# Lemnon95/multithreading_string_matching

Measured on AMD Instinct MI355X. Metric: payload GB/s scanned + matches/s, 1M x 1500B pkts, 1 pattern, higher is better.
Workload: dtype u8; 1 GPU; 1000000 synthetic 1500 B UDP payloads per GPU (a..z, NUL-free, seed 1234), one 16-byte pattern planted in ~10% of packets; BASELINE configs[1]; packets_per_gpu=1000000, payload_len=1500, patterns=1, pattern_len=16, parallelism=packets sharded over 1 GPU(s), all-reduce(SUM) of counts

## Files before the change

multithreading_string_matching_amd/csrc/kmp_dev_common.h:

```cpp
#ifndef KMP_DEV_COMMON_H
#define KMP_DEV_COMMON_H

#include <hip/hip_runtime.h>
#include <stdint.h>

#include "kmp_device.h"

namespace {

constexpr uint32_t ONES  = 0x01010101u;
constexpr uint32_t HIGHS = 0x80808080u;

__device__ __forceinline__ uint32_t zero_byte_mask(uint32_t x) { return (x - ONES) & ~x & HIGHS; }

__device__ __forceinline__ uint32_t wave_shl1(uint32_t v, uint32_t fill)
{
    return (uint32_t)__builtin_amdgcn_update_dpp((int)fill, (int)v, 0x130, 0xF, 0xF, false);
}

__device__ __forceinline__ uint32_t sgpr(uint32_t v) { return (uint32_t)__builtin_amdgcn_readfirstlane((int)v); }

template <bool MASKED>
__device__ __forceinline__ bool is_cand(uint32_t d, uint32_t first, uint32_t mask)
{
    return MASKED ? (((d ^ first) & mask) == 0u) : (d == first);
}
typedef uint32_t u32x4 __attribute__((ext_vector_type(4)));


template <int N>
__device__ __forceinline__ void ring_wait(u32x4 &a, u32x4 &b)
{
    asm volatile("s_waitcnt vmcnt(%2)" : "+v"(a), "+v"(b) : "i"(N) : "memory");
    __builtin_amdgcn_sched_barrier(0);
}

__device__ __forceinline__ void kmp_step(uint32_t ch, uint32_t &j, uint32_t m, const uint8_t *pat,
                                         const uint8_t *fail, uint32_t &cnt)
{
    while (j > 0u && pat[j] != ch) j = fail[j - 1u];
    if (pat[j] == ch) ++j;
    if (j == m) { ++cnt; j = fail[m - 1u]; }
}

__device__ __forceinline__ uint64_t ballot64(bool p) { return __builtin_amdgcn_ballot_w64(p); }

typedef int32_t i32x4 __attribute__((ext_vector_type(4)));

__device__ __forceinline__ i32x4 make_rsrc(const uint8_t *base, uint32_t bytes)
{
    const uint64_t p = reinterpret_cast<uint64_t>(base);
    i32x4 r;
    r.x = (int32_t)sgpr((uint32_t)p);
    r.y = (int32_t)sgpr((uint32_t)(p >> 32) & 0xFFFFu);
    r.z = (int32_t)sgpr(bytes);
    r.w = 0x00020000;
    return r;
}

template <bool NT, bool FRESH = false, bool SAME_REGS = false>
__device__ __forceinline__ void flat_issue(u32x4 &dst, i32x4 rsrc, uint32_t vo, uint32_t so)
{
    if (SAME_REGS) {
        if (NT) asm volatile("s_nop 4\n\tbuffer_load_dwordx4 %0, %1, %2, %3 offen nt" : "+v"(dst) : "v"(vo), "s"(rsrc), "s"(so) : "memory");
        else    asm volatile("s_nop 4\n\tbuffer_load_dwordx4 %0, %1, %2, %3 offen" : "+v"(dst) : "v"(vo), "s"(rsrc), "s"(so) : "memory");
    } else if (FRESH) {
        if (NT) asm volatile("s_nop 4\n\tbuffer_load_dwordx4 %0, %1, %2, %3 offen nt" : "=v"(dst) : "v"(vo), "s"(rsrc), "s"(so) : "memory");
        else    asm volatile("s_nop 4\n\tbuffer_load_dwordx4 %0, %1, %2, %3 offen" : "=v"(dst) : "v"(vo), "s"(rsrc), "s"(so) : "memory");
    } else {
        if (NT) asm volatile("buffer_load_dwordx4 %0, %1, %2, %3 offen nt" : "=v"(dst) : "v"(vo), "s"(rsrc), "s"(so) : "memory");
        else    asm volatile("buffer_load_dwordx4 %0, %1, %2, %3 offen" : "=v"(dst) : "v"(vo), "s"(rsrc), "s"(so) : "memory");
    }
}

struct PatConst {
    uint32_t m;
    uint32_t p[4];
};

__device__ __forceinline__ PatConst load_pat_const(const kmp_pattern_dev *gp)
{
    PatConst pc;
    pc.m = gp->m;
#pragma unroll
    for (int d = 0; d < 4; ++d) pc.p[d] = reinterpret_cast<const uint32_t *>(gp->pat)[d];
    asm volatile("" : "+s"(pc.m), "+s"(pc.p[0]), "+s"(pc.p[1]), "+s"(pc.p[2]), "+s"(pc.p[3]));
    return pc;
}

struct Emitter {
    uint4              *out;
    unsigned long long *counter;
    unsigned long long  cap;
    uint32_t            pattern;
    unsigned long long *marks;
    uint32_t            mark_stride;
    uint32_t            mark_rows;
    const uint2        *windows;
    uint32_t            win_first;
    uint32_t            win_last;
};
static_assert(sizeof(Emitter) % 16 == 0, "the kernel arguments behind the Emitter keep their alignment");

__device__ __forceinline__ void mark_match_as(bool ok, uint64_t pkt, uint32_t pattern, const Emitter &e)
{
    const uint32_t lane = threadIdx.x & 63u;
    uint64_t b = ballot64(ok);
    while (b != 0ull) {
        const uint32_t l = (uint32_t)__builtin_ctzll(b);
        const uint32_t pl = (uint32_t)__builtin_amdgcn_readlane((int)pattern, (int)l);
        const uint32_t klo = (uint32_t)__builtin_amdgcn_readlane((int)(uint32_t)pkt, (int)l);
        const uint32_t khi = (uint32_t)__builtin_amdgcn_readlane((int)(uint32_t)(pkt >> 32), (int)l);
        const uint64_t k = ((uint64_t)khi << 32) | klo;
        b &= ~ballot64(ok && pattern == pl && pkt == k);
        if (lane == l && pl < e.mark_rows && (k >> 6) < e.mark_stride)
            atomicOr(e.marks + (uint64_t)pl * e.mark_stride + (k >> 6), 1ull << (k & 63u));
    }
}

__device__ __forceinline__ void emit_filtered(bool ok, uint64_t pkt, uint32_t offset, uint32_t pattern, const Emitter &e)
{
    if (e.marks) { mark_match_as(ok, pkt, pattern, e); return; }
    const uint64_t b = ballot64(ok);
    if (b == 0ull) return;
    const uint32_t leader = (uint32_t)__builtin_ctzll(b);
    const uint32_t lane = threadIdx.x & 63u;
    unsigned long long base = 0ull;
    if (lane == leader) base = atomicAdd(e.counter, (unsigned long long)__builtin_popcountll(b));
    const uint32_t blo = (uint32_t)__builtin_amdgcn_readlane((int)(uint32_t)base, (int)leader);
    const uint32_t bhi = (uint32_t)__builtin_amdgcn_readlane((int)(uint32_t)(base >> 32), (int)leader);
    if (ok) {
        const uint32_t rank = __builtin_amdgcn_mbcnt_hi((uint32_t)(b >> 32), __builtin_amdgcn_mbcnt_lo((uint32_t)b, 0u));
        const unsigned long long slot = (((unsigned long long)bhi << 32) | blo) + rank;
        if (slot < e.cap) e.out[slot] = make_uint4((uint32_t)pkt, (uint32_t)(pkt >> 32), offset, pattern);
    }
}

template <bool EMIT>
__device__ __forceinline__ void emit_match_as(bool ok, uint64_t pkt, uint32_t offset, uint32_t pattern, const Emitter &e)
{
    if (!EMIT) return;
    if (e.windows) {
        uint2 win = make_uint2(0u, 0u);
        if (ok) win = e.windows[pattern];
        ok = ok && win.x <= offset && offset <= win.y;
    }
    emit_filtered(ok, pkt, offset, pattern, e);
}

template <bool EMIT>
__device__ __forceinline__ void emit_match(bool ok, uint64_t pkt, uint32_t offset, const Emitter &e)
{
    if (!EMIT) return;
    if (e.windows) ok = ok && e.win_first <= offset && offset <= e.win_last;
    emit_filtered(ok, pkt, offset, e.pattern, e);
}

__device__ __forceinline__ int32_t nul_limit(int32_t maxi, const uint32_t (&w)[5], uint64_t zl, uint64_t st, bool dead_in, uint32_t lane)
{
    const uint64_t below = (1ull << lane) - 1ull;
    const uint64_t st_le = st & (below | (1ull << lane));
    bool nul_before;
    if (st_le == 0ull) nul_before = dead_in || ((zl & below) != 0ull);
    else {
        const uint32_t sl = 63u - (uint32_t)__builtin_clzll(st_le);
        nul_before = (zl & below & ~((1ull << sl) - 1ull)) != 0ull;
    }
    const uint32_t m0 = zero_byte_mask(w[0]), m1 = zero_byte_mask(w[1]), m2 = zero_byte_mask(w[2]), m3 = zero_byte_mask(w[3]);
    uint32_t zi = 16u;
    if (m3) zi = 12u + ((uint32_t)__builtin_ctz(m3) >> 3);
    if (m2) zi = 8u + ((uint32_t)__builtin_ctz(m2) >> 3);
    if (m1) zi = 4u + ((uint32_t)__builtin_ctz(m1) >> 3);
    if (m0) zi = (uint32_t)__builtin_ctz(m0) >> 3;
    return nul_before ? -1 : min(maxi, (int32_t)zi - 1);
}

__device__ __forceinline__ uint32_t pk_min_u16(uint32_t a, uint32_t b)
{
    uint32_t r;
    asm("v_pk_min_u16 %0, %1, %2" : "=v"(r) : "v"(a), "v"(b));
    return r;
}
__device__ __forceinline__ uint32_t pk_max_u16(uint32_t a, uint32_t b)
{
    uint32_t r;
    asm("v_pk_max_u16 %0, %1, %2" : "=v"(r) : "v"(a), "v"(b));
    return r;
}
__device__ __forceinline__ uint32_t pk_add_u16(uint32_t a, uint32_t b)
{
    uint32_t r;
    asm("v_pk_add_u16 %0, %1, %2" : "=v"(r) : "v"(a), "v"(b));
    return r;
}
__device__ __forceinline__ uint32_t pk_rsub_sat_u16(uint32_t k, uint32_t b)
{
    uint32_t r;
    asm("v_pk_sub_u16 %0, %1, %2 clamp" : "=v"(r) : "s"(k), "v"(b));
    return r;
}
__device__ __forceinline__ uint32_t zero_half_mask(uint32_t x) { return (x - 0x00010001u) & ~x & 0x80008000u; }

__device__ __forceinline__ uint64_t mqsad(uint32_t lo, uint32_t hi, uint32_t ref, uint64_t acc)
{
    return __builtin_amdgcn_mqsad_pk_u16_u8(((uint64_t)hi << 32) | lo, ref, acc);
}

__device__ __forceinline__ uint32_t filter_sad(const uint32_t (&w)[5], uint32_t first, uint64_t (&S)[4], uint32_t (&t)[4])
{
#pragma unroll
    for (int q = 0; q < 4; ++q) {
        S[q] = mqsad(w[q], w[q + 1], first, 0ull);
        t[q] = pk_min_u16((uint32_t)S[q], (uint32_t)(S[q] >> 32));
    }
    return pk_min_u16(pk_min_u16(t[0], t[1]), pk_min_u16(t[2], t[3]));
}

__device__ __forceinline__ uint32_t halves_product(uint32_t x)
{
    uint32_t r;
    asm("v_mul_u32_u24_sdwa %0, %1, %1 dst_sel:DWORD dst_unused:UNUSED_PAD src0_sel:WORD_0 src1_sel:WORD_1" : "=v"(r) : "v"(x));
    return r;
}

template <bool EMIT>
__device__ __forceinline__ uint32_t tally_group(int q, uint64_t Sq, bool barred, uint32_t nv2, uint32_t found, uint32_t p0, uint32_t &cnt, uint64_t pkt,
                                                const Emitter &em)
{
    uint32_t lo = (uint32_t)Sq, hi = (uint32_t)(Sq >> 32);
    if (barred) {
        asm volatile("" ::: "memory");
        lo = pk_max_u16(lo, pk_rsub_sat_u16((uint32_t)(4 * q + 1) | ((uint32_t)(4 * q + 2) << 16), nv2));
        hi = pk_max_u16(hi, pk_rsub_sat_u16((uint32_t)(4 * q + 3) | ((uint32_t)(4 * q + 4) << 16), nv2));
    }
    if (!EMIT) return pk_add_u16(found, pk_add_u16(pk_rsub_sat_u16(0x00010001u, lo), pk_rsub_sat_u16(0x00010001u, hi)));
#pragma unroll
    for (int a = 0; a < 4; ++a) {
        const bool ok = (((a < 2 ? lo : hi) >> (16 * (a & 1))) & 0xFFFFu) == 0u;
        cnt += ok ? 1u : 0u;
        emit_match<EMIT>(ok, pkt, p0 + (uint32_t)(4 * q + a), em);
    }
    return found;
}

template <int ND, bool EMIT>
__device__ __forceinline__ void confirm_block0(uint64_t (&S)[4], const uint32_t (&t)[4], const uint32_t (&c)[8], bool barred, uint32_t nv2, uint32_t p0,
                                               const PatConst &pc, bool more, uint32_t &cnt, uint64_t pkt, const Emitter &em, bool (&on)[4])
{
    uint32_t found = 0u;
#pragma unroll
    for (int q = 0; q < 4; ++q) {
        on[q] = ballot64(halves_product(t[q]) == 0u) != 0ull;
        if (!on[q]) continue;
        asm volatile("" ::: "memory");
        if (ND > 1) {
            S[q] = mqsad(c[q + 1], c[q + 2], pc.p[1], S[q]);
            S[q] = mqsad(c[q + 2], c[q + 3], pc.p[2], S[q]);
            S[q] = mqsad(c[q + 3], c[q + 4], pc.p[3], S[q]);
        }
        if (more) continue;
        found = tally_group<EMIT>(q, S[q], barred, nv2, found, p0, cnt, pkt, em);
    }
    if (!EMIT) cnt += (found & 0xFFFFu) + (found >> 16);
}

template <bool EMIT>
__device__ __forceinline__ void confirm_sad(uint64_t (&S)[4], const uint32_t (&t)[4], const uint32_t (&w)[5], uint4 v, u32x4 bn, uint32_t fz, int32_t maxi,
                                            uint32_t p0, const PatConst &pc, const kmp_pattern_dev *gp, uint32_t &cnt, uint64_t pkt,
                                            const Emitter &em)
{
    const uint32_t m = pc.m;
    const bool barred = ballot64(maxi < 15 && fz != 0u) != 0ull;
    uint32_t nv2 = 0u;
    if (barred) {
        if (ballot64(maxi >= 0) == 0ull) return;
        const uint32_t nv = (uint32_t)min(max(maxi + 1, 0), 16);
        nv2 = nv | (nv << 16);
    }
    uint32_t c[8] = {w[0], w[1], w[2], w[3], w[4], 0u, 0u, 0u};
    bool on[4];
    if (m <= 4u) { confirm_block0<1, EMIT>(S, t, c, barred, nv2, p0, pc, false, cnt, pkt, em, on); return; }
    c[5] = wave_shl1(v.y, sgpr(bn.y)); c[6] = wave_shl1(v.z, sgpr(bn.z)); c[7] = wave_shl1(v.w, sgpr(bn.w));
    const bool more = m > 16u;
    confirm_block0<4, EMIT>(S, t, c, barred, nv2, p0, pc, more, cnt, pkt, em, on);
    if (!more) return;

    for (uint32_t k = 1u; 16u * k < m; ++k) {
        uint32_t mn = 0xFFFFFFFFu;
#pragma unroll
        for (int q = 0; q < 4; ++q)
            if (on[q]) mn = pk_min_u16(mn, pk_min_u16((uint32_t)S[q], (uint32_t)(S[q] >> 32)));
        if (ballot64(halves_product(mn) == 0u) == 0ull) return;
        const uint4 pk = reinterpret_cast<const uint4 *>(gp->pat)[k];
        const uint32_t left = m - 16u * k;
#pragma unroll
        for (int j = 0; j < 4; ++j) c[j] = c[j + 4];
        c[4] = wave_shl1(c[4], (uint32_t)__builtin_amdgcn_readlane((int)bn.x, (int)k));
        c[5] = wave_shl1(c[5], (uint32_t)__builtin_amdgcn_readlane((int)bn.y, (int)k));
        c[6] = wave_shl1(c[6], (uint32_t)__builtin_amdgcn_readlane((int)bn.z, (int)k));
        c[7] = wave_shl1(c[7], (uint32_t)__builtin_amdgcn_readlane((int)bn.w, (int)k));
#pragma unroll
        for (int q = 0; q < 4; ++q) {
            if (!on[q]) continue;
            asm volatile("" ::: "memory");
            S[q] = mqsad(c[q], c[q + 1], pk.x, S[q]);
            if (left > 4u)  { asm volatile("" ::: "memory"); S[q] = mqsad(c[q + 1], c[q + 2], pk.y, S[q]); }
            if (left > 8u)  { asm volatile("" ::: "memory"); S[q] = mqsad(c[q + 2], c[q + 3], pk.z, S[q]); }
            if (left > 12u) { asm volatile("" ::: "memory"); S[q] = mqsad(c[q + 3], c[q + 4], pk.w, S[q]); }
        }
    }
    uint32_t found = 0u;
#pragma unroll
    for (int q = 0; q < 4; ++q) {
        if (!on[q]) continue;
        asm volatile("" ::: "memory");
        found = tally_group<EMIT>(q, S[q], barred, nv2, found, p0, cnt, pkt, em);
    }
    if (!EMIT) cnt += (found & 0xFFFFu) + (found >> 16);
}


struct kmp_plan_entry { uint64_t k; uint64_t off; };

}

#endif
```

multithreading_string_matching_amd/csrc/kmp_scan_stream.hip:

```cpp
#include <hip/hip_runtime.h>
#include <stdint.h>

#include <algorithm>

#include "kmp_device.h"
#include "kmp_launch.h"
#include "kmp_dev_common.h"

namespace {


__global__ void __launch_bounds__(KMP_BLOCK_THREADS)
kmp_build_bitmap_kernel(const uint64_t *__restrict__ pkt_off, uint64_t n, unsigned long long *__restrict__ bitmap)
{
    for (uint64_t k = (uint64_t)blockIdx.x * blockDim.x + threadIdx.x; k < n; k += (uint64_t)gridDim.x * blockDim.x) {
        const uint64_t slot = pkt_off[k] >> 4;
        atomicOr(bitmap + (slot >> 6), 1ull << (slot & 63ull));
    }
}

__global__ void __launch_bounds__(KMP_BLOCK_THREADS)
kmp_plan_kernel(const uint64_t *__restrict__ pkt_off, const uint32_t *__restrict__ pkt_len, uint64_t n, uint64_t nwaves,
                kmp_plan_shape shape, kmp_plan_entry *__restrict__ plan)
{
    const uint64_t w = (uint64_t)blockIdx.x * blockDim.x + threadIdx.x;
    if (w > nwaves) return;
    const uint64_t l16 = ((uint64_t)pkt_len[n - 1] + 15ull) & ~15ull;
    const uint64_t end = pkt_off[n - 1] + (l16 < 16ull ? 16ull : l16);
    if (w == nwaves) { plan[w].k = n; plan[w].off = end; return; }
    uint64_t target = pkt_off[0];
    if (shape.units == 0u) target += w * shape.step;
    else {
        const uint64_t r = w / shape.units, u = w % shape.units;
        const uint64_t in = u <= shape.big_units ? u * shape.step : shape.big_units * shape.step + (u - shape.big_units) * shape.small;
        target += r * shape.region + (in < shape.region ? in : shape.region);
    }
    uint64_t lo = 0, hi = n;
    while (lo < hi) {
        const uint64_t mid = (lo + hi) >> 1;
        if (pkt_off[mid] < target) lo = mid + 1; else hi = mid;
    }
    if (lo > 0 && w > 0) {
        const uint64_t next = (lo < n) ? pkt_off[lo] : end;
        if (next >= target && target - pkt_off[lo - 1] < next - target) --lo;
    }
    plan[w].k = lo;
    plan[w].off = (lo < n) ? pkt_off[lo] : end;
}

#define KMP_WHOLE false
#define KMP_FLAT_KERNEL kmp_scan_flat_kernel
#define KMP_PACKED_KERNEL kmp_scan_packed_kernel
#include "kmp_scan_stream_kernels.inc"
#undef KMP_WHOLE
#undef KMP_FLAT_KERNEL
#undef KMP_PACKED_KERNEL
#define KMP_WHOLE true
#define KMP_FLAT_KERNEL kmp_scan_flat_whole_kernel
#define KMP_PACKED_KERNEL kmp_scan_packed_whole_kernel
#include "kmp_scan_stream_kernels.inc"
#undef KMP_WHOLE
#undef KMP_FLAT_KERNEL
#undef KMP_PACKED_KERNEL

}

namespace {
Emitter emitter_of(const kmp_scan_args &a)
{
    Emitter e{};
    e.out = reinterpret_cast<uint4 *>(a.emit_out);
    e.counter = a.emit_counter;
    e.cap = a.emit_cap;
    e.pattern = 0;
    e.marks = a.emit_marks;
    e.mark_stride = a.mark_stride;
    e.mark_rows = a.mark_rows;
    e.windows = reinterpret_cast<const uint2 *>(a.emit_windows);
    e.win_first = 0u;
    e.win_last = 0xFFFFFFFFu;
    return e;
}

template <int DEPTH>
hipError_t launch_flat_t(const kmp_scan_args &a, hipStream_t st)
{
    dim3 grid(a.blocks_x, a.n_ids), block(KMP_BLOCK_THREADS);
    const Emitter em = emitter_of(a);
#define KMP_FLAT_ARGS a.arena, a.n_pkts, a.uniform_stride, a.uniform_len, a.pkts_per_wave, a.patterns, a.pat_ids, a.partials, a.zero_counts, em
    if (a.whole) {
        if (kmp_emits(a))
            hipLaunchKernelGGL((kmp_scan_flat_whole_kernel<4, true, true>), grid, block, 0, st, KMP_FLAT_ARGS);
        else if (a.nontemporal)
            hipLaunchKernelGGL((kmp_scan_flat_whole_kernel<4, true>), grid, block, 0, st, KMP_FLAT_ARGS);
        else
            hipLaunchKernelGGL((kmp_scan_flat_whole_kernel<4, false>), grid, block, 0, st, KMP_FLAT_ARGS);
    } else if (kmp_emits(a))
        hipLaunchKernelGGL((kmp_scan_flat_kernel<4, true, true>), grid, block, 0, st, KMP_FLAT_ARGS);
    else if (a.nontemporal)
        hipLaunchKernelGGL((kmp_scan_flat_kernel<DEPTH, true>), grid, block, 0, st, KMP_FLAT_ARGS);
    else
        hipLaunchKernelGGL((kmp_scan_flat_kernel<DEPTH, false>), grid, block, 0, st, KMP_FLAT_ARGS);
#undef KMP_FLAT_ARGS
    return hipGetLastError();
}
}

namespace {
template <int DEPTH>
hipError_t launch_packed_t(const kmp_scan_args &a, hipStream_t st)
{
    dim3 grid(a.blocks_x, a.n_ids), block(KMP_BLOCK_THREADS);
    const kmp_plan_entry *plan = reinterpret_cast<const kmp_plan_entry *>(a.plan);
    const Emitter em = emitter_of(a);
#define KMP_PACKED_ARGS a.arena, a.pkt_off, a.pkt_len, a.bitmap, plan, a.patterns, a.pat_ids, a.partials, a.zero_counts, em, (a.pad_clean ? 1u : 0u)
    if (a.whole) {
        if (kmp_emits(a))
            hipLaunchKernelGGL((kmp_scan_packed_whole_kernel<4, true, true>), grid, block, 0, st, KMP_PACKED_ARGS);
        else if (a.nontemporal)
            hipLaunchKernelGGL((kmp_scan_packed_whole_kernel<4, true>), grid, block, 0, st, KMP_PACKED_ARGS);
        else
            hipLaunchKernelGGL((kmp_scan_packed_whole_kernel<4, false>), grid, block, 0, st, KMP_PACKED_ARGS);
    } else if (kmp_emits(a))
        hipLaunchKernelGGL((kmp_scan_packed_kernel<4, true, true>), grid, block, 0, st, KMP_PACKED_ARGS);
    else if (a.nontemporal)
        hipLaunchKernelGGL((kmp_scan_packed_kernel<DEPTH, true>), grid, block, 0, st, KMP_PACKED_ARGS);
    else
        hipLaunchKernelGGL((kmp_scan_packed_kernel<DEPTH, false>), grid, block, 0, st, KMP_PACKED_ARGS);
#undef KMP_PACKED_ARGS
    return hipGetLastError();
}
}

hipError_t kmp_launch_scan_packed(const kmp_scan_args &a, hipStream_t st)
{
    if (a.n_ids == 0 || a.blocks_x == 0) return hipSuccess;
    switch (a.depth) {
    case 2: case 3: return launch_packed_t<3>(a, st);
    case 6: case 8: return launch_packed_t<6>(a, st);
    default: return launch_packed_t<4>(a, st);
    }
}

hipError_t kmp_launch_build_bitmap(const uint64_t *pkt_off, uint64_t n, unsigned long long *bitmap, hipStream_t st)
{
    if (n == 0) return hipSuccess;
    uint64_t blocks = (n + KMP_BLOCK_THREADS - 1) / KMP_BLOCK_THREADS;
    if (blocks > 4096u) blocks = 4096u;
    hipLaunchKernelGGL(kmp_build_bitmap_kernel, dim3((uint32_t)blocks), dim3(KMP_BLOCK_THREADS), 0, st, pkt_off, n, bitmap);
    return hipGetLastError();
}

hipError_t kmp_launch_plan(const uint64_t *pkt_off, const uint32_t *pkt_len, uint64_t n, uint64_t nwaves, const kmp_plan_shape &shape,
                           void *plan, hipStream_t st)
{
    if (n == 0) return hipSuccess;
    const uint64_t blocks = (nwaves + 1 + KMP_BLOCK_THREADS - 1) / KMP_BLOCK_THREADS;
    hipLaunchKernelGGL(kmp_plan_kernel, dim3((uint32_t)blocks), dim3(KMP_BLOCK_THREADS), 0, st, pkt_off, pkt_len, n, nwaves,
                       shape, reinterpret_cast<kmp_plan_entry *>(plan));
    return hipGetLastError();
}

hipError_t kmp_launch_scan_flat(const kmp_scan_args &a, hipStream_t st)
{
    if (a.n_ids == 0 || a.blocks_x == 0) return hipSuccess;
    switch (a.depth) {
    case 2: return launch_flat_t<2>(a, st);
    case 3: return launch_flat_t<3>(a, st);
    case 5: return launch_flat_t<5>(a, st);
    case 6: return launch_flat_t<6>(a, st);
    case 8: return launch_flat_t<8>(a, st);
    default: return launch_flat_t<4>(a, st);
    }
}
```

multithreading_string_matching_amd/csrc/kmp_scan_stream_kernels.inc:

```


template <int DEPTH, bool NT, bool EMIT = false>
__global__ void __launch_bounds__(KMP_BLOCK_THREADS)
KMP_FLAT_KERNEL(const uint8_t *__restrict__ arena, uint64_t n_pkts, uint32_t stride, uint32_t L,
                uint32_t pkts_per_wave, const kmp_pattern_dev *__restrict__ patterns,
                const uint32_t *__restrict__ pat_ids, unsigned long long *__restrict__ partials, unsigned long long *__restrict__ zero_counts, Emitter em)
{
    __shared__ unsigned long long s_wave_cnt[KMP_BLOCK_WAVES];

    const uint32_t lane = threadIdx.x & (KMP_WAVE - 1u);
    const uint32_t wave = sgpr(threadIdx.x >> 6);
    const uint64_t gw = (uint64_t)blockIdx.x * KMP_BLOCK_WAVES + wave;
    const uint64_t k0 = gw * pkts_per_wave;
    const uint64_t k1 = min(n_pkts, k0 + pkts_per_wave);
    const uint32_t range = (k0 < n_pkts) ? (uint32_t)(k1 - k0) * stride : 0u;
    const uint8_t *base = arena + ((k0 < n_pkts) ? k0 * (uint64_t)stride : 0ull);
    const uint32_t step_mod = KMP_CHUNK % stride;

    const i32x4    rsrc = make_rsrc(base, range);
    const uint32_t vo0 = lane * KMP_LANE_BYTES;
    u32x4 buf[DEPTH];
#pragma unroll
    for (int s = 0; s < DEPTH; ++s) flat_issue<NT, true>(buf[s], rsrc, vo0, (uint32_t)s * KMP_CHUNK);

    const uint32_t pid = pat_ids[blockIdx.y];
    const kmp_pattern_dev *gp = patterns + pid;
    const PatConst pc = load_pat_const(gp);
    const uint32_t m = pc.m;
    if (EMIT) em.pattern = pid;
    if (EMIT && em.windows) {
        const uint2 win = em.windows[pid];
        em.win_first = win.x; em.win_last = win.y;
    }

    uint32_t cnt = 0u;
    {
        uint32_t p0 = vo0 % stride;
        bool     dead = false;
        uint32_t cb = 0u;

        while (cb < range) {
#pragma unroll
            for (int s = 0; s < DEPTH; ++s) {
                ring_wait<DEPTH - 2>(buf[s], buf[(s + 1) % DEPTH]);
                if (cb < range) {
                    const uint4    v   = make_uint4(buf[s].x, buf[s].y, buf[s].z, buf[s].w);
                    const u32x4    bn  = buf[(s + 1) % DEPTH];
                    const uint32_t w[5] = {v.x, v.y, v.z, v.w, wave_shl1(v.x, sgpr(bn.x))};

                    uint64_t S[4];
                    uint32_t t[4];
                    if constexpr (KMP_WHOLE) {
                        const uint32_t fz = zero_half_mask(filter_sad(w, pc.p[0], S, t));
                        if (ballot64(fz != 0u) != 0ull) {
                            int32_t maxi = (int32_t)L - (int32_t)m - (int32_t)p0;
                            if (fz == 0u) maxi = -1;
                            const uint64_t pkt = EMIT ? (k0 + (uint64_t)((cb + vo0 - p0) / stride)) : 0ull;
                            confirm_sad<EMIT>(S, t, w, v, bn, fz, maxi, p0, pc, gp, cnt, pkt, em);
                        }
                    } else {
                    const uint32_t zm = zero_byte_mask(w[0]) | zero_byte_mask(w[1]) | zero_byte_mask(w[2]) | zero_byte_mask(w[3]);
                    const uint32_t fz = zero_half_mask(filter_sad(w, pc.p[0], S, t));
                    const uint64_t zl = ballot64(zm != 0u);
                    const uint64_t st = ballot64(p0 == 0u);
                    const uint64_t cl = ballot64(fz != 0u);
                    const bool dead_in = dead;
                    if (zl == 0ull) { if (st != 0ull) dead = false; }
                    else            dead = (st == 0ull) ? true : ((zl >> (63u - (uint32_t)__builtin_clzll(st))) != 0ull);

                    if (cl != 0ull) {
                        int32_t maxi = (int32_t)L - (int32_t)m - (int32_t)p0;
                        if (fz == 0u) maxi = -1;
                        if (zl != 0ull || dead_in) {
                            const uint64_t last_lanes = ballot64(p0 + KMP_LANE_BYTES == stride);
                            if (dead_in || (zl & ~last_lanes) != 0ull) maxi = nul_limit(maxi, w, zl, st, dead_in, lane);
                            else if (ballot64(zm != 0u && fz != 0u) != 0ull) maxi = nul_limit(maxi, w, 0ull, st, false, lane);
                        }
                        const uint64_t pkt = EMIT ? (k0 + (uint64_t)((cb + vo0 - p0) / stride)) : 0ull;
                        confirm_sad<EMIT>(S, t, w, v, bn, fz, maxi, p0, pc, gp, cnt, pkt, em);
                    }
                    }
                    p0 += step_mod;
                    p0 = min(p0, p0 - stride);
                }
                __builtin_amdgcn_sched_barrier(0);
                flat_issue<NT>(buf[s], rsrc, vo0, cb + (uint32_t)DEPTH * KMP_CHUNK);
                cb += KMP_CHUNK;
            }
        }
#pragma unroll
        for (int s = 0; s < DEPTH; s += 2) ring_wait<0>(buf[s], buf[(s + 1) % DEPTH]);
    }

    unsigned long long c64 = cnt;
#pragma unroll
    for (int o = 32; o > 0; o >>= 1) c64 += __shfl_xor(c64, o);
    if (lane == 0u) s_wave_cnt[wave] = c64;
    __syncthreads();
    if (threadIdx.x == 0u) {
        unsigned long long t = 0ull;
#pragma unroll
        for (uint32_t i = 0; i < KMP_BLOCK_WAVES; ++i) t += s_wave_cnt[i];
        partials[(uint64_t)blockIdx.y * gridDim.x + blockIdx.x] = t;
        if (zero_counts && blockIdx.x == 0u) zero_counts[pid] = 0ull;
    }
}

template <int DEPTH, bool NT, bool EMIT = false>
__global__ void __launch_bounds__(KMP_BLOCK_THREADS)
KMP_PACKED_KERNEL(const uint8_t *__restrict__ arena, const uint64_t *__restrict__ pkt_off,
                  const uint32_t *__restrict__ pkt_len, const unsigned long long *__restrict__ bitmap,
                  const kmp_plan_entry *__restrict__ plan, const kmp_pattern_dev *__restrict__ patterns,
                  const uint32_t *__restrict__ pat_ids, unsigned long long *__restrict__ partials, unsigned long long *__restrict__ zero_counts, Emitter em,
                  uint32_t pad_clean)
{
    __shared__ unsigned long long s_wave_cnt[KMP_BLOCK_WAVES];

    const uint32_t lane = threadIdx.x & (KMP_WAVE - 1u);
    const uint32_t wave = sgpr(threadIdx.x >> 6);
    const uint64_t gw = (uint64_t)blockIdx.x * KMP_BLOCK_WAVES + wave;
    const uint64_t k0 = plan[gw].k, k1 = plan[gw + 1].k;
    const uint64_t off_first = plan[gw].off;
    const uint32_t pre = (uint32_t)(off_first & 127ull), pl = pre >> 4;
    const uint64_t off0 = off_first - pre;
    const uint32_t range = (k1 > k0) ? (uint32_t)(plan[gw + 1].off - off0) : 0u;

    const i32x4    rsrc = make_rsrc(arena + off0, range);
    const uint32_t vo0 = lane * KMP_LANE_BYTES;
    u32x4 buf[DEPTH];
#pragma unroll
    for (int s = 0; s < DEPTH; ++s) flat_issue<NT, true>(buf[s], rsrc, vo0, (uint32_t)s * KMP_CHUNK);

    const uint32_t pid = pat_ids[blockIdx.y];
    const kmp_pattern_dev *gp = patterns + pid;
    const PatConst pc = load_pat_const(gp);
    const uint32_t m = pc.m;
    if (EMIT) em.pattern = pid;
    if (EMIT && em.windows) {
        const uint2 win = em.windows[pid];
        em.win_first = win.x; em.win_last = win.y;
    }

    uint32_t cnt = 0u;
    if (range) {
        const uint64_t b0 = off0 >> 4;
        const unsigned long long *bw = bitmap + (b0 >> 6);
        const uint32_t sh = (uint32_t)(b0 & 63ull);

        unsigned long long hiw[DEPTH];
#pragma unroll
        for (int s = 0; s < DEPTH; ++s) hiw[s] = bw[s + 1];
        unsigned long long low = bw[0];
        uint64_t kbase = k0 - 1ull;
        bool     dead = false;
        uint32_t cb = 0u, j = 0u;

        while (cb < range) {
            uint64_t st_[DEPTH];
#pragma unroll
            for (int s = 0; s < DEPTH; ++s) {
                const unsigned long long hi = hiw[s];
                st_[s] = sh ? ((low >> sh) | (hi << (64u - sh))) : low;
                low = hi;
                asm volatile("" : "+s"(st_[s]));
            }
            __builtin_amdgcn_sched_barrier(0);
#pragma unroll
            for (int s = 0; s < DEPTH; ++s) hiw[s] = bw[j + (uint32_t)DEPTH + 1u + (uint32_t)s];
            __builtin_amdgcn_sched_barrier(0);
#pragma unroll
            for (int s = 0; s < DEPTH; ++s) {
                ring_wait<DEPTH - 2>(buf[s], buf[(s + 1) % DEPTH]);
                if (cb < range) {
                    uint4          v   = make_uint4(buf[s].x, buf[s].y, buf[s].z, buf[s].w);
                    const u32x4    bn  = buf[(s + 1) % DEPTH];
                    uint64_t       st  = st_[s];
                    if (s == 0 && cb == 0u && pl != 0u) {
                        if (lane < pl) v = make_uint4(0u, 0u, 0u, 0u);
                        st &= ~0ull << pl;
                    }
                    const uint32_t w[5] = {v.x, v.y, v.z, v.w, wave_shl1(v.x, sgpr(bn.x))};

                    uint32_t zm = 0u;
                    if constexpr (!KMP_WHOLE) zm = zero_byte_mask(w[0]) | zero_byte_mask(w[1]) | zero_byte_mask(w[2]) | zero_byte_mask(w[3]);
                    uint64_t S[4];
                    uint32_t t[4];
                    const uint32_t fz = zero_half_mask(filter_sad(w, pc.p[0], S, t));
                    uint64_t zl = 0ull;
                    if constexpr (!KMP_WHOLE) zl = ballot64(zm != 0u);
                    const uint64_t cl = ballot64(fz != 0u);
                    const bool dead_in = dead;
                    if constexpr (!KMP_WHOLE) {
                    if (zl == 0ull) { if (st != 0ull) dead = false; }
                    else            dead = (st == 0ull) ? true : ((zl >> (63u - (uint32_t)__builtin_clzll(st))) != 0ull);
                    }

                    if (cl != 0ull) {
                        int32_t  maxi = -1;
                        uint32_t p0 = 0u, L = 0u;
                        uint64_t kl = 0ull;
                        uint64_t nx;
                        if (s + 1 < DEPTH) nx = st_[(s + 1) % DEPTH];
                        else               nx = sh ? ((low >> sh) | (hiw[0] << (64u - sh))) : low;
                        const uint64_t last_lanes = (st >> 1) | (nx << 63);
                        if (!EMIT && pad_clean && m <= 16u && (cl & last_lanes) == 0ull) {
                            maxi = fz != 0u ? 15 : -1;
                        } else if (!EMIT && pad_clean) {
                            if (fz != 0u) {
                                const uint64_t above = (st >> 1) >> lane;
                                uint32_t d = 4096u;
                                if (above != 0ull) d = (uint32_t)__builtin_ctzll(above) + 1u;
                                else if (nx != 0ull) d = 64u - lane + (uint32_t)__builtin_ctzll(nx);
                                L = d * KMP_LANE_BYTES;
                                maxi = (int32_t)L - (int32_t)m;
                            }
                        } else if (fz != 0u) {
                            const uint64_t le = (2ull << lane) - 1ull;
                            kl = kbase + (uint64_t)__builtin_popcountll(st & le);
                            const uint64_t po = pkt_off[kl];
                            L  = pkt_len[kl];
                            p0 = (uint32_t)(off0 + cb + vo0 - po);
                            maxi = (int32_t)L - (int32_t)m - (int32_t)p0;
                        }
                        if constexpr (!KMP_WHOLE) {
                        if (zl != 0ull || dead_in) {
                            if (dead_in || (zl & ~last_lanes) != 0ull) maxi = nul_limit(maxi, w, zl, st, dead_in, lane);
                            else if (ballot64(zm != 0u && fz != 0u) != 0ull) maxi = nul_limit(maxi, w, 0ull, st, false, lane);
                        }
                        }
                        confirm_sad<EMIT>(S, t, w, v, bn, fz, maxi, p0, pc, gp, cnt, kl, em);
                        __builtin_amdgcn_s_waitcnt(0xC07F);
                    }
                    kbase += (uint64_t)__builtin_popcountll(st);
                }
                __builtin_amdgcn_sched_barrier(0);
                flat_issue<NT>(buf[s], rsrc, vo0, cb + (uint32_t)DEPTH * KMP_CHUNK);
                cb += KMP_CHUNK;
                ++j;
            }
        }
    }
#pragma unroll
    for (int s = 0; s < DEPTH; s += 2) ring_wait<0>(buf[s], buf[(s + 1) % DEPTH]);

    unsigned long long c64 = cnt;
#pragma unroll
    for (int o = 32; o > 0; o >>= 1) c64 += __shfl_xor(c64, o);
    if (lane == 0u) s_wave_cnt[wave] = c64;
    __syncthreads();
    if (threadIdx.x == 0u) {
        unsigned long long t = 0ull;
#pragma unroll
        for (uint32_t i = 0; i < KMP_BLOCK_WAVES; ++i) t += s_wave_cnt[i];
        partials[(uint64_t)blockIdx.y * gridDim.x + blockIdx.x] = t;
        if (zero_counts && blockIdx.x == 0u) zero_counts[pid] = 0ull;
    }
}
```

Baseline: 6815 GB/s.

## Restructure SAD confirm path with ballot masks, dense tally, and cheaper NUL limit

Result: no change. 6843 GB/s, median of 3 (+0.4%).

```diff
diff --git a/multithreading_string_matching_amd/csrc/kmp_dev_common.h b/multithreading_string_matching_amd/csrc/kmp_dev_common.h
--- a/multithreading_string_matching_amd/csrc/kmp_dev_common.h
+++ b/multithreading_string_matching_amd/csrc/kmp_dev_common.h
@@ -156,6 +156,14 @@
     emit_filtered(ok, pkt, offset, e.pattern, e);
 }
 
+__device__ __forceinline__ int32_t own_nul_limit(int32_t maxi, const uint32_t (&w)[5], uint32_t n)
+{
+    const uint32_t zlo = __builtin_amdgcn_udot4(zero_byte_mask(w[1]) >> 7, 0x80402010u, __builtin_amdgcn_udot4(zero_byte_mask(w[0]) >> 7, 0x08040201u, 0u, false), false);
+    const uint32_t zhi = __builtin_amdgcn_udot4(zero_byte_mask(w[3]) >> 7, 0x80402010u, __builtin_amdgcn_udot4(zero_byte_mask(w[2]) >> 7, 0x08040201u, 0u, false), false);
+    const uint32_t zb = __builtin_amdgcn_ubfe(zlo | (zhi << 8), 0u, n);
+    return min(maxi, (int32_t)__builtin_ctz(zb | 0x10000u) - 1);
+}
+
 __device__ __forceinline__ int32_t nul_limit(int32_t maxi, const uint32_t (&w)[5], uint64_t zl, uint64_t st, bool dead_in, uint32_t lane)
 {
     const uint64_t below = (1ull << lane) - 1ull;
@@ -166,38 +174,26 @@
         const uint32_t sl = 63u - (uint32_t)__builtin_clzll(st_le);
         nul_before = (zl & below & ~((1ull << sl) - 1ull)) != 0ull;
     }
-    const uint32_t m0 = zero_byte_mask(w[0]), m1 = zero_byte_mask(w[1]), m2 = zero_byte_mask(w[2]), m3 = zero_byte_mask(w[3]);
-    uint32_t zi = 16u;
-    if (m3) zi = 12u + ((uint32_t)__builtin_ctz(m3) >> 3);
-    if (m2) zi = 8u + ((uint32_t)__builtin_ctz(m2) >> 3);
-    if (m1) zi = 4u + ((uint32_t)__builtin_ctz(m1) >> 3);
-    if (m0) zi = (uint32_t)__builtin_ctz(m0) >> 3;
-    return nul_before ? -1 : min(maxi, (int32_t)zi - 1);
-}
-
+    return nul_before ? -1 : own_nul_limit(maxi, w, 16u);
+}
+
+typedef uint16_t u16x2 __attribute__((ext_vector_type(2)));
+__device__ __forceinline__ u16x2 as_u16x2(uint32_t x) { return __builtin_bit_cast(u16x2, x); }
 __device__ __forceinline__ uint32_t pk_min_u16(uint32_t a, uint32_t b)
 {
-    uint32_t r;
-    asm("v_pk_min_u16 %0, %1, %2" : "=v"(r) : "v"(a), "v"(b));
-    return r;
+    return __builtin_bit_cast(uint32_t, __builtin_elementwise_min(as_u16x2(a), as_u16x2(b)));
 }
 __device__ __forceinline__ uint32_t pk_max_u16(uint32_t a, uint32_t b)
 {
-    uint32_t r;
-    asm("v_pk_max_u16 %0, %1, %2" : "=v"(r) : "v"(a), "v"(b));
-    return r;
+    return __builtin_bit_cast(uint32_t, __builtin_elementwise_max(as_u16x2(a), as_u16x2(b)));
 }
 __device__ __forceinline__ uint32_t pk_add_u16(uint32_t a, uint32_t b)
 {
-    uint32_t r;
-    asm("v_pk_add_u16 %0, %1, %2" : "=v"(r) : "v"(a), "v"(b));
-    return r;
+    return __builtin_bit_cast(uint32_t, (u16x2)(as_u16x2(a) + as_u16x2(b)));
 }
 __device__ __forceinline__ uint32_t pk_rsub_sat_u16(uint32_t k, uint32_t b)
 {
-    uint32_t r;
-    asm("v_pk_sub_u16 %0, %1, %2 clamp" : "=v"(r) : "s"(k), "v"(b));
-    return r;
+    return __builtin_bit_cast(uint32_t, __builtin_elementwise_sub_sat(as_u16x2(k), as_u16x2(b)));
 }
 __device__ __forceinline__ uint32_t zero_half_mask(uint32_t x) { return (x - 0x00010001u) & ~x & 0x80008000u; }
 
@@ -243,80 +239,88 @@
     return found;
 }
 
-template <int ND, bool EMIT>
-__device__ __forceinline__ void confirm_block0(uint64_t (&S)[4], const uint32_t (&t)[4], const uint32_t (&c)[8], bool barred, uint32_t nv2, uint32_t p0,
-                                               const PatConst &pc, bool more, uint32_t &cnt, uint64_t pkt, const Emitter &em, bool (&on)[4])
+template <bool EMIT>
+__device__ __forceinline__ void tally_groups(const uint64_t (&S)[4], const uint64_t (&ob)[4], bool dense, bool barred, uint32_t nv2, uint32_t p0,
+                                             uint32_t &cnt, uint64_t pkt, const Emitter &em)
 {
     uint32_t found = 0u;
-#pragma unroll
-    for (int q = 0; q < 4; ++q) {
-        on[q] = ballot64(halves_product(t[q]) == 0u) != 0ull;
-        if (!on[q]) continue;
-        asm volatile("" ::: "memory");
-        if (ND > 1) {
+    if (EMIT) {
+#pragma unroll
+        for (int q = 0; q < 4; ++q) {
+            if (ob[q] == 0ull) continue;
+            asm volatile("" ::: "memory");
+            found = tally_group<EMIT>(q, S[q], barred, nv2, found, p0, cnt, pkt, em);
+        }
+        return;
+    }
+#define KMP_TALLY(DENSE_, BARRED_) do { \
+        asm volatile("" ::: "memory"); \
+        _Pragma("unroll") for (int q = 0; q < 4; ++q) { \
+            if (!(DENSE_)) { if (ob[q] == 0ull) continue; asm volatile("" ::: "memory"); } \
+            found = tally_group<EMIT>(q, S[q], BARRED_, nv2, found, p0, cnt, pkt, em); \
+        } \
+    } while (0)
+    if (dense) { if (barred) KMP_TALLY(true, true); else KMP_TALLY(true, false); }
+    else if (barred) KMP_TALLY(false, true);
+    else KMP_TALLY(false, false);
+#undef KMP_TALLY
+    cnt += (found & 0xFFFFu) + (found >> 16);
+}
+
+template <bool EMIT>
+__device__ __forceinline__ void confirm_sad(uint64_t (&S)[4], const uint32_t (&t)[4], const uint32_t (&w)[5], uint4 v, u32x4 bn, uint64_t cl, int32_t maxi,
+                                            uint32_t p0, const PatConst &pc, const kmp_pattern_dev *gp, uint32_t &cnt, uint64_t pkt,
+                                            const Emitter &em)
+{
+    const uint32_t m = pc.m;
+    const bool barred = (ballot64(maxi < 15) & cl) != 0ull;
+    uint32_t nv2 = 0u;
+    if (barred) {
+        if ((ballot64(maxi >= 0) & cl) == 0ull) return;
+        const uint32_t nv = (uint32_t)min(max(maxi + 1, 0), 16);
+        nv2 = nv | (nv << 16);
+    }
+    uint64_t ob[4];
+    uint32_t hp[4];
+#pragma unroll
+    for (int q = 0; q < 4; ++q) { hp[q] = halves_product(t[q]); ob[q] = ballot64(hp[q] == 0u); }
+    const bool dense = !EMIT && ballot64((hp[0] | hp[1] | hp[2] | hp[3]) == 0u) != 0ull;
+    if (m > 4u) {
+        uint32_t c[8] = {w[0], w[1], w[2], w[3], w[4], wave_shl1(v.y, sgpr(bn.y)), wave_shl1(v.z, sgpr(bn.z)), wave_shl1(v.w, sgpr(bn.w))};
+#pragma unroll
+        for (int q = 0; q < 4; ++q) {
+            if (ob[q] == 0ull) continue;
+            asm volatile("" ::: "memory");
             S[q] = mqsad(c[q + 1], c[q + 2], pc.p[1], S[q]);
             S[q] = mqsad(c[q + 2], c[q + 3], pc.p[2], S[q]);
             S[q] = mqsad(c[q + 3], c[q + 4], pc.p[3], S[q]);
         }
-        if (more) continue;
-        found = tally_group<EMIT>(q, S[q], barred, nv2, found, p0, cnt, pkt, em);
-    }
-    if (!EMIT) cnt += (found & 0xFFFFu) + (found >> 16);
-}
-
-template <bool EMIT>
-__device__ __forceinline__ void confirm_sad(uint64_t (&S)[4], const uint32_t (&t)[4], const uint32_t (&w)[5], uint4 v, u32x4 bn, uint32_t fz, int32_t maxi,
-                                            uint32_t p0, const PatConst &pc, const kmp_pattern_dev *gp, uint32_t &cnt, uint64_t pkt,
-                                            const Emitter &em)
-{
-    const uint32_t m = pc.m;
-    const bool barred = ballot64(maxi < 15 && fz != 0u) != 0ull;
-    uint32_t nv2 = 0u;
-    if (barred) {
-        if (ballot64(maxi >= 0) == 0ull) return;
-        const uint32_t nv = (uint32_t)min(max(maxi + 1, 0), 16);
-        nv2 = nv | (nv << 16);
-    }
-    uint32_t c[8] = {w[0], w[1], w[2], w[3], w[4], 0u, 0u, 0u};
-    bool on[4];
-    if (m <= 4u) { confirm_block0<1, EMIT>(S, t, c, barred, nv2, p0, pc, false, cnt, pkt, em, on); return; }
-    c[5] = wave_shl1(v.y, sgpr(bn.y)); c[6] = wave_shl1(v.z, sgpr(bn.z)); c[7] = wave_shl1(v.w, sgpr(bn.w));
-    const bool more = m > 16u;
-    confirm_block0<4, EMIT>(S, t, c, barred, nv2, p0, pc, more, cnt, pkt, em, on);
-    if (!more) return;
-
-    for (uint32_t k = 1u; 16u * k < m; ++k) {
-        uint32_t mn = 0xFFFFFFFFu;
-#pragma unroll
-        for (int q = 0; q < 4; ++q)
-            if (on[q]) mn = pk_min_u16(mn, pk_min_u16((uint32_t)S[q], (uint32_t)(S[q] >> 32)));
-        if (ballot64(halves_product(mn) == 0u) == 0ull) return;
-        const uint4 pk = reinterpret_cast<const uint4 *>(gp->pat)[k];
-        const uint32_t left = m - 16u * k;
-#pragma unroll
-        for (int j = 0; j < 4; ++j) c[j] = c[j + 4];
-        c[4] = wave_shl1(c[4], (uint32_t)__builtin_amdgcn_readlane((int)bn.x, (int)k));
-        c[5] = wave_shl1(c[5], (uint32_t)__builtin_amdgcn_readlane((int)bn.y, (int)k));
-        c[6] = wave_shl1(c[6], (uint32_t)__builtin_amdgcn_readlane((int)bn.z, (int)k));
-        c[7] = wave_shl1(c[7], (uint32_t)__builtin_amdgcn_readlane((int)bn.w, (int)k));
-#pragma unroll
-        for (int q = 0; q < 4; ++q) {
-            if (!on[q]) continue;
-            asm volatile("" ::: "memory");
-            S[q] = mqsad(c[q], c[q + 1], pk.x, S[q]);
-            if (left > 4u)  { asm volatile("" ::: "memory"); S[q] = mqsad(c[q + 1], c[q + 2], pk.y, S[q]); }
-            if (left > 8u)  { asm volatile("" ::: "memory"); S[q] = mqsad(c[q + 2], c[q + 3], pk.z, S[q]); }
-            if (left > 12u) { asm volatile("" ::: "memory"); S[q] = mqsad(c[q + 3], c[q + 4], pk.w, S[q]); }
+        for (uint32_t k = 1u; 16u * k < m; ++k) {
+            uint32_t mn = pk_min_u16((uint32_t)S[0], (uint32_t)(S[0] >> 32));
+#pragma unroll
+            for (int q = 1; q < 4; ++q) mn = pk_min_u16(mn, pk_min_u16((uint32_t)S[q], (uint32_t)(S[q] >> 32)));
+            if (ballot64(halves_product(mn) == 0u) == 0ull) return;
+            const uint4 pk = reinterpret_cast<const uint4 *>(gp->pat)[k];
+            const uint32_t left = m - 16u * k;
+#pragma unroll
+            for (int j = 0; j < 4; ++j) c[j] = c[j + 4];
+            c[4] = wave_shl1(c[4], (uint32_t)__builtin_amdgcn_readlane((int)bn.x, (int)k));
+            c[5] = wave_shl1(c[5], (uint32_t)__builtin_amdgcn_readlane((int)bn.y, (int)k));
+            c[6] = wave_shl1(c[6], (uint32_t)__builtin_amdgcn_readlane((int)bn.z, (int)k));
+            c[7] = wave_shl1(c[7], (uint32_t)__builtin_amdgcn_readlane((int)bn.w, (int)k));
+#pragma unroll
+            for (int q = 0; q < 4; ++q) {
+                if (ob[q] == 0ull) continue;
+                asm volatile("" ::: "memory");
+                S[q] = mqsad(c[q], c[q + 1], pk.x, S[q]);
+                if (left > 4u)  { asm volatile("" ::: "memory"); S[q] = mqsad(c[q + 1], c[q + 2], pk.y, S[q]); }
+                if (left > 8u)  { asm volatile("" ::: "memory"); S[q] = mqsad(c[q + 2], c[q + 3], pk.z, S[q]); }
+                if (left > 12u) { asm volatile("" ::: "memory"); S[q] = mqsad(c[q + 3], c[q + 4], pk.w, S[q]); }
+            }
         }
     }
-    uint32_t found = 0u;
-#pragma unroll
-    for (int q = 0; q < 4; ++q) {
-        if (!on[q]) continue;
-        asm volatile("" ::: "memory");
-        found = tally_group<EMIT>(q, S[q], barred, nv2, found, p0, cnt, pkt, em);
-    }
-    if (!EMIT) cnt += (found & 0xFFFFu) + (found >> 16);
+    asm volatile("" : "+s"(ob[0]), "+s"(ob[1]), "+s"(ob[2]), "+s"(ob[3]));
+    tally_groups<EMIT>(S, ob, dense, barred, nv2, p0, cnt, pkt, em);
 }
 
 
diff --git a/multithreading_string_matching_amd/csrc/kmp_scan_stream.hip b/multithreading_string_matching_amd/csrc/kmp_scan_stream.hip
--- a/multithreading_string_matching_amd/csrc/kmp_scan_stream.hip
+++ b/multithreading_string_matching_amd/csrc/kmp_scan_stream.hip
@@ -87,7 +87,8 @@
 {
     dim3 grid(a.blocks_x, a.n_ids), block(KMP_BLOCK_THREADS);
     const Emitter em = emitter_of(a);
-#define KMP_FLAT_ARGS a.arena, a.n_pkts, a.uniform_stride, a.uniform_len, a.pkts_per_wave, a.patterns, a.pat_ids, a.partials, a.zero_counts, em
+    const uint32_t pad_short = (a.pad_clean && a.uniform_len < a.uniform_stride) ? 1u : 0u;
+#define KMP_FLAT_ARGS a.arena, a.n_pkts, a.uniform_stride, a.uniform_len, a.pkts_per_wave, a.patterns, a.pat_ids, a.partials, a.zero_counts, em, pad_short
     if (a.whole) {
         if (kmp_emits(a))
             hipLaunchKernelGGL((kmp_scan_flat_whole_kernel<4, true, true>), grid, block, 0, st, KMP_FLAT_ARGS);
diff --git a/multithreading_string_matching_amd/csrc/kmp_scan_stream_kernels.inc b/multithreading_string_matching_amd/csrc/kmp_scan_stream_kernels.inc
--- a/multithreading_string_matching_amd/csrc/kmp_scan_stream_kernels.inc
+++ b/multithreading_string_matching_amd/csrc/kmp_scan_stream_kernels.inc
@@ -4,7 +4,8 @@
 __global__ void __launch_bounds__(KMP_BLOCK_THREADS)
 KMP_FLAT_KERNEL(const uint8_t *__restrict__ arena, uint64_t n_pkts, uint32_t stride, uint32_t L,
                 uint32_t pkts_per_wave, const kmp_pattern_dev *__restrict__ patterns,
-                const uint32_t *__restrict__ pat_ids, unsigned long long *__restrict__ partials, unsigned long long *__restrict__ zero_counts, Emitter em)
+                const uint32_t *__restrict__ pat_ids, unsigned long long *__restrict__ partials, unsigned long long *__restrict__ zero_counts, Emitter em,
+                uint32_t pad_short)
 {
     __shared__ unsigned long long s_wave_cnt[KMP_BLOCK_WAVES];
 
@@ -33,6 +34,7 @@
         em.win_first = win.x; em.win_last = win.y;
     }
 
+    [[maybe_unused]] const bool own_moot = pad_short && m + (stride - L) >= 16u;
     uint32_t cnt = 0u;
     {
         uint32_t p0 = vo0 % stride;
@@ -52,11 +54,11 @@
                     uint32_t t[4];
                     if constexpr (KMP_WHOLE) {
                         const uint32_t fz = zero_half_mask(filter_sad(w, pc.p[0], S, t));
-                        if (ballot64(fz != 0u) != 0ull) {
-                            int32_t maxi = (int32_t)L - (int32_t)m - (int32_t)p0;
-                            if (fz == 0u) maxi = -1;
+                        const uint64_t cl = ballot64(fz != 0u);
+                        if (cl != 0ull) {
+                            const int32_t maxi = pad_short ? 15 : (int32_t)L - (int32_t)m - (int32_t)p0;
                             const uint64_t pkt = EMIT ? (k0 + (uint64_t)((cb + vo0 - p0) / stride)) : 0ull;
-                            confirm_sad<EMIT>(S, t, w, v, bn, fz, maxi, p0, pc, gp, cnt, pkt, em);
+                            confirm_sad<EMIT>(S, t, w, v, bn, cl, maxi, p0, pc, gp, cnt, pkt, em);
                         }
                     } else {
                     const uint32_t zm = zero_byte_mask(w[0]) | zero_byte_mask(w[1]) | zero_byte_mask(w[2]) | zero_byte_mask(w[3]);
@@ -69,15 +71,15 @@
                     else            dead = (st == 0ull) ? true : ((zl >> (63u - (uint32_t)__builtin_clzll(st))) != 0ull);
 
                     if (cl != 0ull) {
-                        int32_t maxi = (int32_t)L - (int32_t)m - (int32_t)p0;
-                        if (fz == 0u) maxi = -1;
+                        int32_t maxi = pad_short ? 15 : (int32_t)L - (int32_t)m - (int32_t)p0;
                         if (zl != 0ull || dead_in) {
                             const uint64_t last_lanes = ballot64(p0 + KMP_LANE_BYTES == stride);
                             if (dead_in || (zl & ~last_lanes) != 0ull) maxi = nul_limit(maxi, w, zl, st, dead_in, lane);
-                            else if (ballot64(zm != 0u && fz != 0u) != 0ull) maxi = nul_limit(maxi, w, 0ull, st, false, lane);
+                            else if (!own_moot && (zl & cl) != 0ull)
+                                maxi = own_nul_limit(maxi, w, pad_short ? min(L - min(L, p0), 16u) : 16u);
                         }
                         const uint64_t pkt = EMIT ? (k0 + (uint64_t)((cb + vo0 - p0) / stride)) : 0ull;
-                        confirm_sad<EMIT>(S, t, w, v, bn, fz, maxi, p0, pc, gp, cnt, pkt, em);
+                        confirm_sad<EMIT>(S, t, w, v, bn, cl, maxi, p0, pc, gp, cnt, pkt, em);
                     }
                     }
                     p0 += step_mod;
@@ -225,10 +227,10 @@
                         if constexpr (!KMP_WHOLE) {
                         if (zl != 0ull || dead_in) {
                             if (dead_in || (zl & ~last_lanes) != 0ull) maxi = nul_limit(maxi, w, zl, st, dead_in, lane);
-                            else if (ballot64(zm != 0u && fz != 0u) != 0ull) maxi = nul_limit(maxi, w, 0ull, st, false, lane);
-                        }
-                        }
-                        confirm_sad<EMIT>(S, t, w, v, bn, fz, maxi, p0, pc, gp, cnt, kl, em);
+                            else if ((zl & cl) != 0ull) maxi = own_nul_limit(maxi, w, 16u);
+                        }
+                        }
+                        confirm_sad<EMIT>(S, t, w, v, bn, cl, maxi, p0, pc, gp, cnt, kl, em);
                         __builtin_amdgcn_s_waitcnt(0xC07F);
                     }
                     kbase += (uint64_t)__builtin_popcountll(st);
```
